# griosd/g3py

Hardware: AMD Instinct MI355X
Metric: GP logp+predict end-to-end (Gram+Cholesky+solves), N=32768 fp64: algorithmic TFLOP/s (higher is better)
Workload: dtype f64; 1 GPU; SE-kernel GaussianProcess, N=32768 d=4, M=1024 test points: Gram + blocked Cholesky + L^-1 y (logp) + cross-Gram + 1024-rhs trsm + posterior mean/variance; N=32768, d=4, M=1024, parallelism=1gpu

## Files before the change

### g3py_amd/csrc/g3_api.hip

```cpp
#include "g3_internal.h"
#include "g3_host.h"
#include <stdlib.h>

extern "C" int g3_version(void) { return 102; }

static int ctx_create_impl(int device, hipStream_t on_stream, g3_ctx** out);
extern "C" int g3_ctx_create(int device, g3_ctx** out) { return ctx_create_impl(device, nullptr, out); }
int g3i_ctx_create_on(int device, hipStream_t stream, g3_ctx** out) { return stream ? ctx_create_impl(device, stream, out) : -3; }
#include <time.h>
__global__ void probe_long_kernel(int iters) {
  for (int i = 0; i < iters; ++i) __builtin_amdgcn_s_sleep(127);
}
__global__ void probe_tiny_kernel(unsigned* out) {
  if (threadIdx.x == 0 && out) *out = 1u;
}
static double probe_now_us() {
  struct timespec ts;
  clock_gettime(CLOCK_MONOTONIC, &ts);
  return (double)ts.tv_sec * 1e6 + (double)ts.tv_nsec * 1e-3;
}
bool g3i_probe_pair(hipStream_t a, hipStream_t b, unsigned* scratch, double* tiny_us, double* long_us, int reps) {
  double best = 1e30, lbest = 1e30;
  for (int rep = 0; rep < reps; ++rep) {
    if (hipStreamSynchronize(a) != hipSuccess || hipStreamSynchronize(b) != hipSuccess) return false;
// ... 648 lines not shown
                          const void* delta, g3_dtype dt, void* K, int64_t ldk, void* invd, void* a, double out[6],
                          const g3_kernel_prog* prog_cross, const void* Xs, int64_t M, int64_t ldxs, void* mu,
                          void* ss) {
  const int64_t Np = g3_roundup(N, G3_LB), RB = 128, Mp = M > 0 ? g3_roundup(M, 128) : 0;
  const int64_t E = RB + Mp;
  const size_t es = g3_esize(dt);
  const double es_d = (double)es;
  char* rhs = (char*)K + (size_t)Np * ldk * es;
  char* Vp = rhs + (size_t)RB * ldk * es;
  int rc = G3_OK;
  const unsigned gflags = G3_GRAM_LOWER | G3_GRAM_SCRUB | G3_GRAM_PAD_EYE;
  auto build_rhs = [&]() -> int {
    const int r0 = pad_row_launch(ctx, rhs, ldk, delta, N, Np, RB, dt);
    if (r0) return r0;
    if (M > 0) {
      const int pr = g3i_prof_begin(ctx, G3_TAG_CROSS_GRAM, (double)(N + M) * d * es_d + (double)N * M * es_d);
      int r = g3_gram(ctx, prog_cross, Xs, M, ldxs, X, N, ldx, d, dt, Vp, ldk, Mp, Np, G3_GRAM_SCRUB);
      g3i_prof_end(ctx, pr);
      if (r) return r;
    }
    return G3_OK;
  };
  auto build = [&]() -> int {
    const int pr = g3i_prof_begin(ctx, G3_TAG_GRAM, (double)N * d * es_d + 0.5 * (double)N * (N + 1) * es_d);
    int r = g3_gram(ctx, prog, X, N, ldx, nullptr, 0, 0, d, dt, K, ldk, Np, Np, gflags);
    if (r) return r;
    r = g3_cov_lift(ctx, K, N, ldk, dt);
    g3i_prof_end(ctx, pr);
    if (r) return r;
    return build_rhs();
  };
  auto factor = [&]() -> int {
    const int pr = g3i_prof_begin(ctx, G3_TAG_POTRF, (double)N * N * N / 3.0 + (double)N * N * (1 + M));
    const int r = g3i_potrf_tall(ctx, K, Np, ldk, dt, invd, E);
    g3i_prof_end(ctx, pr);
    return r;
  };
  double st4[5];
  auto finish = [&]() -> int {
    const int pr = g3i_prof_begin(ctx, G3_TAG_REDUCE, 2.0 * N * M);
    g3_by_dtype(dt, [&](auto t) {
      using T = decltype(t);
      hipLaunchKernelGGL((logp_finish_kernel<T>), dim3(1), dim3(1024), 0, ctx->stream, (const T*)K, N, Np, ldk, (const T*)rhs, (T*)a,
                         ctx->d_stats, ctx->d_info);
    });
    G3_LAUNCH_CHECK();
    int r = G3_OK;
    if (M > 0 && (mu || ss)) r = rows_dot_ss_launch(ctx, Vp, M, N, ldk, a, dt, mu, ss);
    g3i_prof_end(ctx, pr);
    if (r) return r;
    r = fetch_stats(ctx, st4, 5);
    if (!r) { ctx->info_clean = true; ctx->info_sync = true; }
    return r;
  };
  rc = build();
  if (rc) return rc;
  rc = factor();
  if (rc) return rc;
  rc = finish();
  if (rc) return rc;
  int info = (int)st4[4];
  double tries = 0, fallback = 0;
  const int info0 = info;
  if (info != 0) {
    rc = build();
    if (rc) return rc;
// ... 118 lines not shown
  if (!a) return -15;
  if (!out) return -16;
  g3_kernel_prog first;
  if (g3i_validate_members(mp, batch, d, &first)) return -2;
  if (batch == 1)
    return gp_factor_impl(ctx, &first, X, N, ldx, d, delta, dt, K, ldk, invd, a, out, nullptr, nullptr, 0, 0, nullptr,
                          nullptr);
  const size_t sbytes = (size_t)batch * 4 * sizeof(double);
  g3_dev_members dm;
  int rc = g3i_upload_members(ctx, mp, batch, sbytes, g3i_coop_ctl_bytes(batch), &dm);
  if (rc) return rc;
  double* dstats = dm.stats;
  const int64_t wstride = Np * G3_LB;
  char* rhs = (char*)K + (size_t)Np * ldk * es;
  const bool small = Np <= 2 * G3_LB;
  int pr = g3i_prof_begin(ctx, G3_TAG_GRAM, (double)batch * ((double)N * d + 0.5 * (double)N * (N + 1)) * es);
  rc = g3i_gram_batched(ctx, dm.progs, &first, batch, X, N, ldx, d, dt, K, ldk, kstride, Np,
                        G3_GRAM_LOWER | G3_GRAM_SCRUB | G3_GRAM_PAD_EYE);
  if (!rc) rc = diag_stats_launch(ctx, K, N, ldk, dt, nullptr, 1, batch, kstride);
  if (!rc && !small) rc = pad_row_launch(ctx, rhs, ldk, delta, N, Np, RB, dt, batch, kstride, ldd);
  g3i_prof_end(ctx, pr);
  if (rc) return rc;
  pr = g3i_prof_begin(ctx, G3_TAG_POTRF, (double)batch * ((double)N * N * N / 3.0 + (double)N * N));
  if (small) {
    rc = g3i_small_factor_batched(ctx, K, ldk, kstride, invd, wstride, delta, ldd, a, Np, dstats, batch, N, Np, dt);
    g3i_prof_end(ctx, pr);
    if (!rc) rc = read_member_flags(ctx, batch, false);
  } else if (Np <= ctx->tune.coop_max_n && batch >= ctx->tune.coop_min_batch) {
    rc = g3i_coop_factor_batched(ctx, K, ldk, kstride, invd, wstride, (unsigned*)dm.tail, batch, Np, dt);
    g3i_prof_end(ctx, pr);
    if (!rc) rc = read_member_flags(ctx, batch, false);
  } else {
    g3_batch_scope mode(ctx, batch, kstride, wstride, invd, (size_t)batch * wstride * es);
    rc = g3i_potrf_tall(ctx, K, Np, ldk, dt, invd, RB);
    g3i_prof_end(ctx, pr);
    if (!rc) rc = read_member_flags(ctx, batch, true);
  }
  if (rc) return rc;
  if (!small) {
    G3_HIP(hipMemcpy2DAsync(a, (size_t)Np * es, rhs, (size_t)kstride * es, (size_t)Np * es, (size_t)batch,
                            hipMemcpyDeviceToDevice, ctx->stream));
    rc = g3i_logp_terms_dev(ctx, K, N, ldk, a, dt, dstats, batch, kstride, Np);
    if (rc) return rc;
  }
  double* hst = (double*)malloc(sbytes);
  if (!hst) return G3_ERR_NOMEM;
  if (hipMemcpyAsync(hst, dstats, sbytes, hipMemcpyDeviceToHost, ctx->stream) != hipSuccess ||
      hipStreamSynchronize(ctx->stream) != hipSuccess) {
    free(hst);
    snprintf(ctx->err, sizeof(ctx->err), "g3_gp_factor_batched: statistics copy failed");
    return G3_ERR_HIP;
  }
  int* infos = (int*)malloc(sizeof(int) * batch);
  if (!infos) { free(hst); return G3_ERR_NOMEM; }
  memcpy(infos, ctx->h_info, sizeof(int) * batch);
  for (int b = 0; b < batch && !rc; ++b) {
    double* o = out + 6 * b;
    if (infos[b] == 0) {
      o[0] = hst[4 * b]; o[1] = hst[4 * b + 1]; o[2] = hst[4 * b + 2];
      o[3] = 0; o[4] = 0; o[5] = 0;
    } else {
      g3_kernel_prog mine;
      mp.member(b, &mine);
      rc = gp_factor_impl(ctx, &mine, X, N, ldx, d, (const char*)delta + (size_t)b * ldd * es, dt,
                          (char*)K + (size_t)b * kstride * es, ldk, (char*)invd + (size_t)b * wstride * es,
                          (char*)a + (size_t)b * Np * es, o, nullptr, nullptr, 0, 0, nullptr, nullptr);
// ... 435 lines not shown
```

### g3py_amd/csrc/g3_gemm.hip

```cpp
#include "g3_internal.h"
#include <stdlib.h>

#include "g3_mfma.h"
#include "g3_host.h"

#include "g3_gemm_tile.h"


template <typename T, int BM, int BN, int WM, int WN, int NSTAGE>
__global__ void __launch_bounds__((BM / WM) * (BN / WN) * 64, ((BM / WM) * (BN / WN) >= 16 ? 1 : 2))
gemm_nt_kernel(T* C, int64_t ldc, const T* A, int64_t lda, const T* B, int64_t ldb,
               int K, T alpha, T beta, const int* __restrict__ info,
               int64_t bsC, int64_t bsA, int64_t bsB, const RasterTab tab) {
  C += (int64_t)blockIdx.y * bsC;
  A += (int64_t)blockIdx.y * bsA;
  B += (int64_t)blockIdx.y * bsB;
  if (info != nullptr) info += blockIdx.y;

  int bm, bn;
  {
    const int nwg = gridDim.x, id = blockIdx.x;
    const int q = nwg >> 3, r = nwg & 7, xcd = id & 7;
    const int v = (xcd < r ? xcd * (q + 1) : r * (q + 1) + (xcd - r) * q) + (id >> 3);
    int lo = 0, hi = tab.ngroups;
    while (hi - lo > 1) {
      const int mid = (lo + hi) >> 1;
      if (tab.g[mid].prefix <= v) lo = mid; else hi = mid;
    }
    const int w = v - tab.g[lo].prefix;
    const int rows = (int)tab.g[lo].nrows;
    bn = w / rows;
    bm = (int)tab.g[lo].row0 + (w - bn * rows);
  }
  const int doff = tab.diag_off;
  const bool lower_only = doff < G3_DENSE_OFF;
  const int m0 = bm * BM, n0 = bn * BN;
  if (lower_only && n0 > m0 + BM - 1 + doff) return;
  const int failed = (info != nullptr) ? *info : 0;
  int64_t brow = n0;
  if (tab.b_nb > 0) {
    const int sblk = n0 / tab.b_nb;
    brow = (int64_t)tab.b_blk[sblk] * tab.b_nb + (n0 - sblk * tab.b_nb);
  }
  extern __shared__ __attribute__((aligned(16))) char smem[];
  const int Kt = (tab.k_tri && n0 + BN < K) ? n0 + BN : K;
  gemm_tile<T, BM, BN, WM, WN, NSTAGE>(C, ldc, A + (int64_t)m0 * lda, lda, B + brow * ldb, ldb, Kt, alpha, beta, m0, n0,
                                       lower_only, doff, failed, smem);
}

template <typename T, int BM>
__global__ void __launch_bounds__(256, 2)
trsm_stripe_kernel(T* X, int64_t ldx, const T* L, int64_t ldl, const T* W, const int* __restrict__ info,
                   int64_t bsX, int64_t bsL, int64_t bsW, const TrsmOps ops) {
  X += (int64_t)blockIdx.y * bsX;
  L += (int64_t)blockIdx.y * bsL;
  W += (int64_t)blockIdx.y * bsW;
  if (info != nullptr) info += blockIdx.y;
  const int failed = (info != nullptr) ? *info : 0;
  if (failed != 0) return;
  extern __shared__ __attribute__((aligned(16))) char smem[];
  const int m0 = blockIdx.x * BM;
  for (int i = 0; i < ops.nops; ++i) {
    const auto o = ops.op[i];
    const T* gB = o.leaf ? W + (int64_t)o.brow * G3_LB * G3_LB : L + (int64_t)o.brow * ldl + o.bcol;
    gemm_tile<T, BM, 128, BM, 32, STAGES>(X, ldx, X + (int64_t)m0 * ldx + o.acol, ldx, gB, o.leaf ? (int64_t)G3_LB : ldl, o.k,
                                          o.leaf ? T(1) : T(-1), o.leaf ? T(0) : T(1), m0, o.col, false, G3_DENSE_OFF, 0, smem);
    __syncthreads();
  }
}


template <typename T, int BM, int BN, int WM, int WN, int NSTAGE>
static int launch_cfg(g3_ctx* ctx, void* C, int64_t ldc, const void* A, int64_t lda, const void* B,
                      int64_t ldb, int64_t k, double alpha, double beta, const GemmShape& sh) {
  constexpr int NT = (BM / WM) * (BN / WN) * 64;
  constexpr int LDS = NSTAGE * (BM + BN) * ROWB;
  auto kern = gemm_nt_kernel<T, BM, BN, WM, WN, NSTAGE>;
  static bool attr_set[G3_MAX_DEVICES] = {};
  const int dev_slot = ctx->device & (G3_MAX_DEVICES - 1);
  if (!attr_set[dev_slot]) {
    G3_HIP(hipFuncSetAttribute(reinterpret_cast<const void*>(kern),
                               hipFuncAttributeMaxDynamicSharedMemorySize, 160 * 1024));
    attr_set[dev_slot] = true;
  }
  RasterTab tab;
  const long long nv = build_raster<BM, BN>(sh, &tab);
  if (nv < 0) {
    snprintf(ctx->err, sizeof(ctx->err), "GEMM raster needs more than %d row groups", G3_RASTER_MAX);
    return G3_ERR_HIP;
  }
  if (nv == 0) return G3_OK;
  dim3 grid((unsigned)nv, (unsigned)g3_nbatch(ctx));
  int lds_req = LDS;
  if (ctx->tune.side_lds > LDS && (g3_on_bulk_stream(ctx) || ctx->bulk_role)) lds_req = ctx->tune.side_lds;
  const int tag = (BM == 128 && BN == 128) ? (nv >= 4096 ? G3_TAG_GEMM_BIG : G3_TAG_GEMM_MID) : G3_TAG_GEMM_SMALL;
  const double kmean = sh.k_tri ? 0.5 * ((double)k + (double)BN) : (double)k;
  const int pr = g3i_prof_begin(ctx, tag, 2.0 * shape_elems(sh) * kmean);
  if (FILE* lg = ctx->gemm_log)
    fprintf(lg, "gemm %d %d %d %lld %lld %lld %d %lld %.9e %d\n", BM, BN, NT / 64, (long long)sh.m, (long long)sh.n, (long long)k, sh.kind,
            nv, 2.0 * shape_elems(sh) * kmean, g3_on_bulk_stream(ctx) ? 1 : 0);
  hipLaunchKernelGGL(kern, grid, dim3(NT), lds_req, ctx->stream, (T*)C, ldc, (const T*)A, lda,
                     (const T*)B, ldb, (int)k, (T)alpha, (T)beta, ctx->d_info,
                     g3_bstride_of(ctx, C), g3_bstride_of(ctx, A), g3_bstride_of(ctx, B), tab);
  g3i_prof_end(ctx, pr);
  G3_LAUNCH_CHECK();
  return G3_OK;
}

template <typename T>
static int launch_t(g3_ctx* ctx, void* C, int64_t ldc, const void* A, int64_t lda, const void* B,
                    int64_t ldb, int64_t k, double alpha, double beta, const GemmShape& sh, int wide) {
  const int64_t blocks128 = (int64_t)(shape_elems(sh) / (128.0 * 128.0)) * g3_nbatch(ctx);
  bool all128 = sh.m % 128 == 0 && sh.n % 128 == 0;
  if (sh.kind == 2)
    for (int s = 0; s < sh.nseg; ++s) all128 = all128 && sh.seg_rows[s] % 128 == 0 && sh.seg_cols[s] % 128 == 0;
  if (wide) {
    if (sh.kind == 0 && sh.n % 128 == 0 && sh.m % 32 == 0)
      return launch_cfg<T, 32, 128, 32, 32, STAGES>(ctx, C, ldc, A, lda, B, ldb, k, alpha, beta, sh);
    snprintf(ctx->err, sizeof(ctx->err), "in-place panel GEMM needs n %% 128 == 0 and m %% 32 == 0 (m=%lld n=%lld)",
             (long long)sh.m, (long long)sh.n);
    return G3_ERR_HIP;
  }
  const int64_t big_min = ctx->tune.gemm_big_min;
  if (all128 && (blocks128 >= big_min || (blocks128 >= ctx->tune.gemm_big_min_k && k >= 1024 && big_min == 4096)))
    return launch_cfg<T, 128, 128, 64, 32, STAGES>(ctx, C, ldc, A, lda, B, ldb, k, alpha, beta, sh);
  return launch_cfg<T, 64, 64, 32, 32, STAGES>(ctx, C, ldc, A, lda, B, ldb, k, alpha, beta, sh);
}

static int launch_dt(g3_ctx* ctx, void* C, int64_t ldc, const void* A, int64_t lda, const void* B,
                     int64_t ldb, int64_t k, double alpha, double beta, g3_dtype dt, const GemmShape& sh, int wide) {
  return g3_by_dtype(dt, [&](auto t) { return launch_t<decltype(t)>(ctx, C, ldc, A, lda, B, ldb, k, alpha, beta, sh, wide); });
}

int g3i_gemm_nt_ex(g3_ctx* ctx, void* C, int64_t ldc, const void* A, int64_t lda, const void* B,
                   int64_t ldb, int64_t m, int64_t n, int64_t k, double alpha, double beta,
                   g3_dtype dt, int lower_only, int wide) {
  if (m == 0 || n == 0) return G3_OK;
  const GemmShape sh{lower_only ? 1 : 0, m, n, 0, 0, nullptr, nullptr, 0, nullptr, 0, nullptr, 0};
  return launch_dt(ctx, C, ldc, A, lda, B, ldb, k, alpha, beta, dt, sh, wide);
}

int g3i_gemm_nt(g3_ctx* ctx, void* C, int64_t ldc, const void* A, int64_t lda, const void* B,
                int64_t ldb, int64_t m, int64_t n, int64_t k, double alpha, double beta,
                g3_dtype dt, int lower_only) {
  return g3i_gemm_nt_ex(ctx, C, ldc, A, lda, B, ldb, m, n, k, alpha, beta, dt, lower_only, 0);
}

int g3i_gemm_nt_ktri(g3_ctx* ctx, void* C, int64_t ldc, const void* A, int64_t lda, const void* V, int64_t ldv, int64_t m, int64_t n,
                     double alpha, double beta, g3_dtype dt) {
  if (m == 0 || n == 0) return G3_OK;
  const GemmShape sh{0, m, n, 0, 0, nullptr, nullptr, 0, nullptr, 0, nullptr, 1};
  return launch_dt(ctx, C, ldc, A, lda, V, ldv, n, alpha, beta, dt, sh, 0);
}

int g3i_gemm_nt_trap(g3_ctx* ctx, void* C, int64_t ldc, const void* A, int64_t lda, const void* B,
                     int64_t ldb, int64_t m, int64_t n, int64_t k, double alpha, double beta,
                     g3_dtype dt, int64_t diag_off) {
  if (m == 0 || n == 0) return G3_OK;
  const GemmShape sh{1, m, n, diag_off, 0, nullptr, nullptr, 0, nullptr, 0, nullptr, 0};
  return launch_dt(ctx, C, ldc, A, lda, B, ldb, k, alpha, beta, dt, sh, 0);
}

template <typename T, int BM>
static int trsm_stripe_t(g3_ctx* ctx, const T* L, int64_t n, int64_t ldl, T* X, int64_t m, int64_t ldx, const T* W) {
  constexpr int LDS = STAGES * (BM + 128) * ROWB;
  auto kern = trsm_stripe_kernel<T, BM>;
  static bool attr_set[G3_MAX_DEVICES] = {};
  const int dev_slot = ctx->device & (G3_MAX_DEVICES - 1);
  if (!attr_set[dev_slot]) {
    G3_HIP(hipFuncSetAttribute(reinterpret_cast<const void*>(kern), hipFuncAttributeMaxDynamicSharedMemorySize, LDS));
    attr_set[dev_slot] = true;
  }
  TrsmOps ops;
  ops.nops = 0;
  trsm_ops_rec(&ops, 0, n);
  const int pr = g3i_prof_begin(ctx, G3_TAG_GEMM_SMALL, (double)m * (double)n * (double)n);
  if (FILE* lg = ctx->gemm_log)
    fprintf(lg, "trsm %d 128 4 %lld %lld %lld 0 %lld %.9e %d\n", BM, (long long)m, (long long)n, (long long)n, (long long)(m / BM),
            (double)m * (double)n * (double)n, g3_on_bulk_stream(ctx) ? 1 : 0);
  hipLaunchKernelGGL(kern, dim3((unsigned)(m / BM), (unsigned)g3_nbatch(ctx)), dim3(256), LDS, ctx->stream, X, ldx, L, ldl, W,
                     ctx->d_info, g3_bstride_of(ctx, X), g3_bstride_of(ctx, L), g3_bstride_of(ctx, W), ops);
  g3i_prof_end(ctx, pr);
  G3_LAUNCH_CHECK();
  return G3_OK;
}

int g3i_trsm_stripe(g3_ctx* ctx, const void* L, int64_t n, int64_t ldl, void* X, int64_t m, int64_t ldx, const void* W,
                    g3_dtype dt) {
  if (n > 1024 || n % G3_LB || m % 32 || m <= 0) return 1;
  const int64_t al = 16 / (int64_t)g3_esize(dt);
  if (ldx % al || ldl % al || (((uintptr_t)X | (uintptr_t)L | (uintptr_t)W) & 15)) return 1;
  const int64_t thin_max = ctx->tune.trsm_thin_max;
// ... 90 lines not shown
```

### g3py_amd/csrc/g3_host.h

```cpp
#pragma once
#include <stddef.h>
#include <stdint.h>
#include <stdlib.h>
#include <string.h>

#include <vector>

#include "g3hip.h"

#define G3H_LB 128

static inline int64_t g3h_roundup(int64_t n, int64_t m) { return (n + m - 1) / m * m; }

static inline int g3h_env_int(const char* name, int dflt) {
  const char* e = getenv(name);
  return e ? atoi(e) : dflt;
}

struct G3hTune {
  int64_t nb;
  int sb;
  int nb_tail;
  int nb_min;
  int nb_head;
  int side_lds;
  int64_t gemm_big_min;
  int64_t gemm_big_min_k;
  int64_t trsm_thin_max;
  int64_t trsm_wide_min;
  int64_t trsm_split_min;
  int64_t trsm_split_n;
  int stair_max;
  int gram_interpret;
  int grad_interpret;
  int gram_jit;
  int coop_max_n;
  int coop_min_batch;
  int coop_group;
  int probe;
};
#define G3H_STAIR_MAX 160
static inline G3hTune g3h_tune_from_env() {
  G3hTune t;
  const char* e = getenv("G3_NB");
  t.nb = e ? atoll(e) : 0;
  t.sb = g3h_env_int("G3_SB", 1);
  t.nb_tail = g3h_env_int("G3_NB_TAIL", 10);
  t.nb_min = g3h_env_int("G3_NB_MIN", 128);
  t.nb_head = g3h_env_int("G3_NB_HEAD", -1);
  t.side_lds = g3h_env_int("G3_SIDE_LDS", 54000);
  e = getenv("G3_GEMM_BIG_MIN");
  t.gemm_big_min = e ? atoll(e) : 4096;
  e = getenv("G3_GEMM_BIG_MIN_K");
  t.gemm_big_min_k = e ? atoll(e) : 1024;
  e = getenv("G3_TRSM_THIN_MAX");
  t.trsm_thin_max = e ? atoll(e) : 2048;
  e = getenv("G3_TRSM_WIDE_MIN");
  t.trsm_wide_min = e ? atoll(e) : 12288;
  e = getenv("G3_TRSM_SPLIT_MIN");
  t.trsm_split_min = e ? atoll(e) : 0;
  e = getenv("G3_TRSM_SPLIT_N");
  t.trsm_split_n = e ? atoll(e) : 512;
  const int sm = g3h_env_int("G3_STAIR_MAX", G3H_STAIR_MAX);
  t.stair_max = sm < 1 ? 1 : (sm > G3H_STAIR_MAX ? G3H_STAIR_MAX : sm);
  t.gram_interpret = g3h_env_int("G3_GRAM_NOFAST", 0) ? 1 : 0;
  t.grad_interpret = g3h_env_int("G3_GRAD_GENERIC", 0) ? 1 : 0;
  t.gram_jit = g3h_env_int("G3_GRAM_JIT", 1) ? 1 : 0;
  t.coop_max_n = g3h_env_int("G3_COOP_MAX_N", 1024);
  t.coop_min_batch = g3h_env_int("G3_COOP_MIN_BATCH", 200);
  t.coop_group = g3h_env_int("G3_COOP_GROUP", 0);
  t.probe = g3h_env_int("G3_PROBE", 1);
  return t;
}

static inline void g3h_panel_bounds(int64_t n, int64_t NB, int G, int batch, const G3hTune& tune, std::vector<int64_t>* bnd, std::vector<int>* grp) {
  const int taper = tune.nb_tail;
  const int wmin = tune.nb_min;
  const int64_t wlo = batch > 1 && wmin < 256 ? 256 : wmin;
  bnd->clear();
  grp->clear();
  if (NB < G3H_LB) NB = G3H_LB;
  if (G < 1) G = 1;
  const int head = tune.nb_head >= 0 ? tune.nb_head : (n <= 16384 ? 1 : 0);
  int64_t r0 = 0;
  int hstep = head;
  while (r0 < n) {
    int64_t w = NB;
    if (hstep > 0 && n >= 8 * NB) {
      w = NB >> hstep;
      if (w < G3H_LB) w = G3H_LB;
      --hstep;
    }
    if (taper) {
      const int64_t rem = n - r0;
      while (w > wlo && rem <= (int64_t)taper * w) w /= 2;
    }
    w = g3h_roundup(w, G3H_LB);
    bnd->push_back(r0);
    r0 += w;
  }
  bnd->push_back(n);
  const int nblk = (int)bnd->size() - 1;
  for (int k = 0; k < nblk; k += G) grp->push_back(k);
  grp->push_back(nblk);
}

constexpr int GROUP_M = 4;
constexpr int G3_RASTER_MAX = 160;
constexpr int G3_DENSE_OFF = 1 << 30;
struct RasterTab {
  int ngroups;
  int diag_off;
  struct Group {
    int prefix;
    unsigned short row0;
    unsigned short nrows;
  } g[G3_RASTER_MAX + 1];
  int b_nb;
  unsigned short b_blk[G3_RASTER_MAX];
  int k_tri;
};


struct GemmShape {
  int kind;
  int64_t m, n;
  int64_t off;
  int nseg;
  const int64_t* seg_rows;
  const int64_t* seg_cols;
  int64_t b_nb;
  const int32_t* b_perm;
  int nperm;
  const int64_t* seg_diag;
  int k_tri;
};

static inline double shape_elems(const GemmShape& sh) {
  if (sh.kind == 0) return (double)sh.m * (double)sh.n;
  if (sh.kind == 2) {
    double e = 0;
    for (int s = 0; s < sh.nseg; ++s) {
      e += (double)sh.seg_rows[s] * (double)sh.seg_cols[s];
      if (sh.seg_diag && sh.seg_diag[s] && sh.seg_cols[s] >= sh.seg_rows[s])
        e -= 0.5 * (double)sh.seg_rows[s] * ((double)sh.seg_rows[s] - 1.0);
    }
    return e;
  }
  int64_t i0 = sh.off < 0 ? -sh.off : 0;
  if (i0 > sh.m) i0 = sh.m;
  int64_t i1 = sh.n - 1 - sh.off;
  if (i1 < i0) i1 = i0;
  if (i1 > sh.m) i1 = sh.m;
  const double cnt = (double)(i1 - i0);
  const double tri = cnt * ((double)i0 + (double)sh.off + 1.0) + 0.5 * cnt * (cnt - 1.0);
  return tri + (double)(sh.m - i1) * (double)sh.n;
}

template <int BM, int BN>
static inline long long build_raster(const GemmShape& sh, RasterTab* tab) {
  const int64_t tiles_m = sh.m / BM;
  tab->diag_off = sh.kind == 1 ? (int)sh.off : G3_DENSE_OFF;
  int ng = 0;
  long long total = 0;
  auto push = [&](int64_t row_tile0, int64_t rows, int64_t nc) -> bool {
    if (rows <= 0 || nc <= 0) return true;
    if (ng >= G3_RASTER_MAX) return false;
    tab->g[ng].prefix = (int)total;
    tab->g[ng].row0 = (unsigned short)row_tile0;
    tab->g[ng].nrows = (unsigned short)rows;
    total += rows * nc;
    ++ng;
    return true;
  };
  if (sh.kind == 2) {
    int64_t rt = 0;
    int64_t ngroups_min = 0;
    for (int s = 0; s < sh.nseg; ++s) ngroups_min += (sh.seg_rows[s] / BM + GROUP_M - 1) / GROUP_M;
    const int64_t gh = ngroups_min <= G3_RASTER_MAX ? GROUP_M : GROUP_M * ((ngroups_min + G3_RASTER_MAX - 1) / G3_RASTER_MAX + 1);
    for (int s = 0; s < sh.nseg; ++s) {
      const int64_t st = sh.seg_rows[s] / BM, nc = sh.seg_cols[s] / BN;
      const bool dg = sh.seg_diag && sh.seg_diag[s] && sh.seg_cols[s] >= sh.seg_rows[s];
      const int64_t dcol0 = sh.seg_cols[s] - sh.seg_rows[s];
      for (int64_t t = 0; t < st; t += gh) {
        const int64_t rows = st - t < gh ? st - t : gh;
        int64_t ncg = nc;
        if (dg) {
          ncg = (dcol0 + (t + rows) * BM - 1) / BN + 1;
          if (ncg > nc) ncg = nc;
        }
        if (!push(rt + t, rows, ncg)) return -1;
      }
      rt += st;
    }
  } else {
    const int64_t tiles_n = sh.n / BN;
    int64_t gh = GROUP_M;
    if ((tiles_m + gh - 1) / gh > G3_RASTER_MAX) gh = (tiles_m + G3_RASTER_MAX - 1) / G3_RASTER_MAX;
    if (gh > 65535) return -1;
    for (int64_t t = 0; t < tiles_m; t += gh) {
      const int64_t rows = tiles_m - t < gh ? tiles_m - t : gh;
      int64_t nc = tiles_n;
      if (sh.kind == 1) {
        const int64_t lim = (t + rows) * BM - 1 + sh.off;
        nc = lim < 0 ? 0 : lim / BN + 1;
        if (nc > tiles_n) nc = tiles_n;
      }
      if (!push(t, rows, nc)) return -1;
    }
  }
  tab->ngroups = ng;
  tab->g[ng].prefix = (int)total;
  tab->g[ng].row0 = 0;
  tab->g[ng].nrows = 1;
  tab->k_tri = (sh.kind == 0 && sh.k_tri) ? 1 : 0;
  tab->b_nb = 0;
  if (sh.b_nb > 0 && sh.b_perm) {
    if (sh.nperm > G3_RASTER_MAX || sh.b_nb % BN) return -1;
    tab->b_nb = (int)sh.b_nb;
    for (int i = 0; i < sh.nperm; ++i) tab->b_blk[i] = (unsigned short)sh.b_perm[i];
  }
  return total;
}


constexpr int G3_TRSM_MAXOPS = 20;
struct TrsmOps {
  int nops;
  struct Op {
    int col;
    int acol;
    int k;
    int brow, bcol;
    int leaf;
  } op[G3_TRSM_MAXOPS];
};


static inline int64_t g3h_split_point(int64_t n) {
  int64_t g = G3H_LB;
  while (g * 2 <= n / 4 && g < 2048) g *= 2;
// ... 325 lines not shown
```

### g3py_amd/csrc/g3_internal.h

```cpp
#pragma once
#include <hip/hip_runtime.h>
#include <stdint.h>
#include <stdio.h>
#include <string.h>

#include "g3hip.h"
#include "g3_host.h"
#include "g3_reduce.h"

#define G3_LB 128

#define G3_PROG_SLOTS 8
struct g3_ctx {
  int device;
  hipStream_t stream;
  hipStream_t own_stream;
  hipStream_t side_stream;
  hipStream_t side_for;
  hipEvent_t* la_ev;
  int la_nev;
  bool in_sweep;
  G3hTune tune;
  unsigned long long gram_paths[3];
  unsigned long long grad_paths[3];
  FILE* gemm_log;
  bool info_clean;
  bool info_sync;
  hipStream_t info_stream;
  bool adopted;
  bool bulk_role;
  int batch;
  int64_t bstride, bstride_w;
  const char* bw_base;
  size_t bw_bytes;
  int64_t gram_diag_off;
  void* bbuf;
  size_t bbuf_bytes;
  int* d_info;
  double* d_stats;
  g3_kernel_prog* d_prog;
  hipEvent_t prog_ev[G3_PROG_SLOTS];
  bool prog_busy[G3_PROG_SLOTS];
  int prog_next, prog_last;
  hipStream_t prog_stream;
  int* h_info;
  double* h_stats;
  g3_kernel_prog* h_prog;
  void* invd;
  size_t invd_bytes;
  void* work;
  size_t work_bytes;
  bool prof_on;
  int prof_level;
  unsigned prof_skip;
  hipEvent_t* prof_ev;
  int prof_cap, prof_n;
  struct { int e0, e1, tag; double work; }* prof_rec;
  int prof_nrec;
  char err[512];
};

enum { G3_TAG_GEMM_BIG = 0, G3_TAG_GRAM = 1, G3_TAG_POTRF = 2, G3_TAG_TRSV = 3, G3_TAG_CROSS_GRAM = 4,
       G3_TAG_TRSM = 5, G3_TAG_REDUCE = 6, G3_TAG_GEMM_MID = 7, G3_TAG_GEMM_SMALL = 8, G3_TAG_LEAF = 9,
// ... 31 lines not shown
  ~g3_dev_guard() {
    if (switched && prev >= 0) (void)hipSetDevice(prev);
  }
  g3_dev_guard(const g3_dev_guard&) = delete;
  g3_dev_guard& operator=(const g3_dev_guard&) = delete;
};
#define G3_MAX_DEVICES 64

#define G3_MAX_BATCH 4096
static inline int g3_nbatch(const g3_ctx* ctx) { return ctx->batch > 1 ? ctx->batch : 1; }
static inline int64_t g3_bstride_of(const g3_ctx* ctx, const void* p) {
  if (ctx->batch <= 1) return 0;
  const char* c = (const char*)p;
  return (ctx->bw_base && c >= ctx->bw_base && c < ctx->bw_base + ctx->bw_bytes) ? ctx->bstride_w : ctx->bstride;
}

struct g3_batch_scope {
  g3_ctx* ctx;
  g3_batch_scope(g3_ctx* c, int batch, int64_t stride, int64_t stride_w, const void* w_base, size_t w_bytes) : ctx(c) {
    ctx->batch = batch;
    ctx->bstride = stride;
    ctx->bstride_w = stride_w;
    ctx->bw_base = (const char*)w_base;
    ctx->bw_bytes = w_bytes;
  }
  ~g3_batch_scope() {
    ctx->batch = 0;
    ctx->bw_base = nullptr;
  }
  g3_batch_scope(const g3_batch_scope&) = delete;
  g3_batch_scope& operator=(const g3_batch_scope&) = delete;
};

static inline bool g3_on_bulk_stream(const g3_ctx* ctx) { return ctx->stream == ctx->side_stream; }

int g3i_ensure_events(g3_ctx* ctx, int need);

struct g3_stream_scope {
  g3_ctx* ctx;
  hipStream_t prev;
  g3_stream_scope(g3_ctx* c, hipStream_t s) : ctx(c), prev(c->stream) { ctx->stream = s; }
  ~g3_stream_scope() { ctx->stream = prev; }
  g3_stream_scope(const g3_stream_scope&) = delete;
  g3_stream_scope& operator=(const g3_stream_scope&) = delete;
};

struct g3_sweep_scope {
  g3_ctx* ctx;
  hipStream_t chain, bulk;
  hipEvent_t ev;
  int rc;
  g3_sweep_scope(g3_ctx* c, hipStream_t bulk_, hipEvent_t ev_) : ctx(c), chain(c->stream), bulk(bulk_), ev(ev_) {
    if (bulk != chain) ctx->in_sweep = true;
    rc = wait(bulk, chain);
  }
  ~g3_sweep_scope() {
    if (bulk != chain) ctx->in_sweep = false;
  }
  int join() { return wait(chain, bulk); }
  g3_sweep_scope(const g3_sweep_scope&) = delete;
  g3_sweep_scope& operator=(const g3_sweep_scope&) = delete;

 private:
  int wait(hipStream_t waiter, hipStream_t on) {
    if (bulk == chain) return G3_OK;
    G3_HIP(hipEventRecord(ev, on));
    G3_HIP(hipStreamWaitEvent(waiter, ev, 0));
    return G3_OK;
  }
};

static inline size_t g3_esize(g3_dtype dt) { return dt == G3_F64 ? 8 : 4; }
static inline int64_t g3_roundup(int64_t n, int64_t m) { return (n + m - 1) / m * m; }

template <typename F>
static inline auto g3_by_dtype(g3_dtype dt, F&& f) {
  if (dt == G3_F64) return f(double());
  return f(float());
}

int g3i_ctx_create_on(int device, hipStream_t stream, g3_ctx** out);
int g3i_ensure_side_stream(g3_ctx* ctx);
void g3i_ctx_forget_stream(g3_ctx* ctx, hipStream_t s);
bool g3i_probe_pair(hipStream_t a, hipStream_t b, unsigned* scratch, double* tiny_us, double* long_us, int reps);

int g3i_gemm_nt(g3_ctx* ctx, void* C, int64_t ldc, const void* A, int64_t lda, const void* B,
                int64_t ldb, int64_t m, int64_t n, int64_t k, double alpha, double beta,
                g3_dtype dt, int lower_only);
int g3i_gemm_nt_ex(g3_ctx* ctx, void* C, int64_t ldc, const void* A, int64_t lda, const void* B,
                   int64_t ldb, int64_t m, int64_t n, int64_t k, double alpha, double beta,
                   g3_dtype dt, int lower_only, int wide);
int g3i_gemm_nt_ktri(g3_ctx* ctx, void* C, int64_t ldc, const void* A, int64_t lda, const void* V, int64_t ldv, int64_t m, int64_t n,
                     double alpha, double beta, g3_dtype dt);
int g3i_gemm_nt_trap(g3_ctx* ctx, void* C, int64_t ldc, const void* A, int64_t lda, const void* B,
                     int64_t ldb, int64_t m, int64_t n, int64_t k, double alpha, double beta,
                     g3_dtype dt, int64_t diag_off);
int g3i_gemm_nt_stair(g3_ctx* ctx, void* C, int64_t ldc, const void* A, int64_t lda, const void* B,
                      int64_t ldb, int64_t k, const int64_t* seg_rows, const int64_t* seg_cols, int nseg,
                      double alpha, double beta, g3_dtype dt, int64_t b_nb, const int32_t* b_perm, int nperm,
                      const int64_t* seg_diag = nullptr);
int g3i_trsm_stripe(g3_ctx* ctx, const void* L, int64_t n, int64_t ldl, void* X, int64_t m, int64_t ldx, const void* W,
                    g3_dtype dt);
int g3i_potrf(g3_ctx* ctx, void* A, int64_t n, int64_t ld, g3_dtype dt, void* invd);
int g3i_potrf_tall(g3_ctx* ctx, void* A, int64_t n, int64_t ld, g3_dtype dt, void* invd, int64_t E);
int g3i_trsm_rlt(g3_ctx* ctx, const void* L, int64_t n, int64_t ldl, void* B, int64_t m,
                 int64_t ldb, g3_dtype dt, const void* invd);
int g3i_trtri_blocks(g3_ctx* ctx, const void* L, int64_t n, int64_t ldl, g3_dtype dt, void* invd);
int g3i_trtri_full(g3_ctx* ctx, const void* L, int64_t n, const void* W, void* V, void* Vt, void* U, g3_dtype dt);
int g3i_reset_info(g3_ctx* ctx);
int g3i_read_info(g3_ctx* ctx, int* info_host);
bool g3i_info_known_zero(const g3_ctx* ctx);
int g3i_diag_stats_dev(g3_ctx* ctx, const void* A, int64_t n, int64_t ld, g3_dtype dt, double* out_dev);
int g3i_logp_terms_dev(g3_ctx* ctx, const void* L, int64_t n, int64_t ld, const void* a, g3_dtype dt, double* out_dev, int batch = 1,
                       int64_t lstride = 0, int64_t astride = 0);
int g3i_small_factor_batched(g3_ctx* ctx, void* K, int64_t ld, int64_t kstride, void* W, int64_t wstride, const void* delta, int64_t ldd,
                             void* a, int64_t astride, double* dstats, int batch, int64_t n, int64_t np, g3_dtype dt);
size_t g3i_coop_ctl_bytes(int batch);
int g3i_coop_group(const g3_ctx* ctx, int batch, int64_t np);
int g3i_coop_factor_batched(g3_ctx* ctx, void* K, int64_t ld, int64_t kstride, void* W, int64_t wstride, unsigned* ctl, int batch,
                            int64_t np, g3_dtype dt);
int g3i_diag_add(g3_ctx* ctx, void* A, int64_t n, int64_t ld, g3_dtype dt, double value);
int g3i_scale(g3_ctx* ctx, void* A, int64_t rows, int64_t cols, int64_t ld, g3_dtype dt, double factor);
int g3i_gram_grad(g3_ctx* ctx, const g3_kernel_prog* prog, const g3_grad_map* map, const void* X, int64_t N, int64_t ldx,
                  int d, g3_dtype dt, const void* G, int64_t ldg, const void* alpha, double* out_host,
                  int64_t row0 = 0, int64_t nrows = -1);
#define G3_GRAD_JIT_MAXSLOTS 40
hipFunction_t g3i_grad_jit_function(g3_ctx* ctx, const g3_kernel_prog* prog_host, int d, g3_dtype dt, int* nslots);
int g3i_gram_grad_batched(g3_ctx* ctx, const g3_kernel_prog* progs, int batch, const g3_grad_map* map, const void* X, int64_t N,
                          int64_t ldx, int d, g3_dtype dt, const void* G, int64_t ldg, int64_t gstride, const void* alpha,
// ... 63 lines not shown
```

### g3py_amd/csrc/g3_potrf.hip

```cpp
#include "g3_internal.h"
#include <vector>
#include "g3_host.h"
#include "g3_mfma.h"
#include "g3_gemm_tile.h"
#include <stdlib.h>

#include "g3_diag.h"

template <typename T>
__global__ void __launch_bounds__(512, 4)
potrf256_kernel(T* A, int64_t ld, T* W, int* info, int64_t row_base, int64_t a_batch, int64_t w_batch) {
  info += blockIdx.y;
  if (*info != 0) return;
  A += (int64_t)blockIdx.y * a_batch;
  W += (int64_t)blockIdx.y * w_batch;
  __shared__ DiagLds<T> S;
  const int lane = threadIdx.x & 63;
  const int wv = __builtin_amdgcn_readfirstlane((int)(threadIdx.x >> 6));
  const int w = wv < 4 ? wv : 11 - wv;
  switch (w) {
    case 0: potrf256_wave<T, 0>(A, ld, W, info, row_base, S, lane); break;
    case 1: potrf256_wave<T, 1>(A, ld, W, info, row_base, S, lane); break;
    case 2: potrf256_wave<T, 2>(A, ld, W, info, row_base, S, lane); break;
    case 3: potrf256_wave<T, 3>(A, ld, W, info, row_base, S, lane); break;
// ... 226 lines not shown
  ctx->work_bytes = bytes;
  return G3_OK;
}


template <typename T>
static int potrf_lookahead(g3_ctx* ctx, T* A, int64_t n, int64_t ld, T* W, int64_t NB, int G, g3_dtype dt, int64_t E) {
  const int64_t R = n + E;
  std::vector<int64_t> bnd;
  std::vector<int> gb;
  g3h_panel_bounds(n, NB, G, ctx->batch, ctx->tune, &bnd, &gb);
  const int nblk = (int)bnd.size() - 1, ngrp = (int)gb.size() - 1;
  int rc = g3i_ensure_events(ctx, 4 * ngrp + 1);
  if (rc) return rc;
  hipEvent_t* evG = ctx->la_ev;
  hipEvent_t* evB1 = ctx->la_ev + ngrp;
  hipEvent_t* evB2a = ctx->la_ev + 2 * ngrp;
  rc = g3i_ensure_side_stream(ctx);
  if (rc) return rc;
  hipStream_t sA = ctx->stream, sB = ctx->side_stream;
  auto r = [&](int k) { return k < nblk ? bnd[k] : n; };
  auto c = [&](int s) { return s < ngrp ? bnd[gb[s]] : n; };
  g3_sweep_scope sweep(ctx, sB, ctx->la_ev[4 * ngrp]);
  if (sweep.rc) return sweep.rc;
  auto panel = [&](int k) -> int {
    T* Akk = A + r(k) * ld + r(k);
    const int64_t w = r(k + 1) - r(k);
    int e = potrf_rec<T>(ctx, Akk, w, ld, W + (r(k) / LB) * LB * LB, r(k), dt);
    if (e) return e;
    if (r(k + 1) < R) e = trsm_rec<T>(ctx, Akk, w, ld, A + r(k + 1) * ld + r(k), R - r(k + 1), ld,
                                      W + (r(k) / LB) * LB * LB, dt);
    return e;
  };
  auto update = [&](int64_t row0, int64_t col0, int64_t col1, int64_t k0, int64_t k1) -> int {
    if (col1 <= col0 || row0 >= R || k1 <= k0) return G3_OK;
    return g3i_gemm_nt_trap(ctx, A + row0 * ld + col0, ld, A + row0 * ld + k0, ld, A + col0 * ld + k0, ld, R - row0,
                            col1 - col0, k1 - k0, -1.0, 1.0, dt, row0 - col0);
  };
  for (int s = 0; s < ngrp; ++s) {
    const int g0 = gb[s], g1 = gb[s + 1];
    if (s >= 1) {
      if (s >= 2) G3_HIP(hipStreamWaitEvent(sA, evB2a[s - 2], 0));
      rc = update(r(g0), r(g0), r(g0 + 1), c(s - 1), c(s));
      if (rc) return rc;
    }
    for (int j = g0; j < g1; ++j) {
      rc = panel(j);
      if (rc) return rc;
      if (j + 1 < g1) {
        if (j == g0 && s >= 1) G3_HIP(hipStreamWaitEvent(sA, evB1[s - 1], 0));
        rc = update(r(j + 1), r(j + 1), r(j + 2), r(j), r(j + 1));
        if (!rc && j + 2 < g1) rc = update(r(j + 2), r(j + 2), c(s + 1), r(j), r(j + 1));
        if (rc) return rc;
      }
    }
    G3_HIP(hipEventRecord(evG[s], sA));
    if (c(s + 1) < n) {
      G3_HIP(hipStreamWaitEvent(sB, evG[s], 0));
      g3_stream_scope on_bulk(ctx, sB);
      const int h0 = gb[s + 1];
      rc = update(r(h0 + 1), r(h0 + 1), c(s + 2), c(s), c(s + 1));
      if (rc) return rc;
      G3_HIP(hipEventRecord(evB1[s], sB));
      if (c(s + 2) < n) {
        const int q0 = gb[s + 2];
        rc = update(c(s + 2), c(s + 2), r(q0 + 1), c(s), c(s + 1));
        if (rc) return rc;
        G3_HIP(hipEventRecord(evB2a[s], sB));
        rc = update(r(q0 + 1), r(q0 + 1), n, c(s), c(s + 1));
        if (rc) return rc;
// ... 422 lines not shown
```

Baseline: 62.70 TFLOP/s.

## Use thin 16-row GEMM tiles for the single-row RHS block in tall Cholesky updates

During the tall Cholesky factorization the appended right-hand-side rows (at row n) only hold one live row, yet trailing updates computed a full 128-row tile band for them. The raster builder now carves that band out into thin 16-row tiles placed at the end of each XCD's schedule, and these are computed with a dedicated 16xBN gemm_tile path. This drops the wasted FLOPs and loads on the padded RHS rows. The cost is added raster/scheduling complexity and a non-inlined thin tile path, and it relies on only the first 16 of the 128 padded rows needing results.

Result: no change. 63.20 TFLOP/s (median of 6 runs) (+0.8%).

```diff
diff --git a/g3py_amd/csrc/g3_api.hip b/g3py_amd/csrc/g3_api.hip
--- a/g3py_amd/csrc/g3_api.hip
+++ b/g3py_amd/csrc/g3_api.hip
@@ -704,6 +704,7 @@
   };
   auto factor = [&]() -> int {
     const int pr = g3i_prof_begin(ctx, G3_TAG_POTRF, (double)N * N * N / 3.0 + (double)N * N * (1 + M));
+    g3_rhs_one_row_scope one_row(ctx);
     const int r = g3i_potrf_tall(ctx, K, Np, ldk, dt, invd, E);
     g3i_prof_end(ctx, pr);
     return r;
@@ -888,6 +889,7 @@
     if (!rc) rc = read_member_flags(ctx, batch, false);
   } else {
     g3_batch_scope mode(ctx, batch, kstride, wstride, invd, (size_t)batch * wstride * es);
+    g3_rhs_one_row_scope one_row(ctx);
     rc = g3i_potrf_tall(ctx, K, Np, ldk, dt, invd, RB);
     g3i_prof_end(ctx, pr);
     if (!rc) rc = read_member_flags(ctx, batch, true);
diff --git a/g3py_amd/csrc/g3_gemm.hip b/g3py_amd/csrc/g3_gemm.hip
--- a/g3py_amd/csrc/g3_gemm.hip
+++ b/g3py_amd/csrc/g3_gemm.hip
@@ -6,6 +6,13 @@
 
 #include "g3_gemm_tile.h"
 
+
+template <typename T, int BN, int NSTAGE>
+__device__ __noinline__ void gemm_tile_thin(T* C, int64_t ldc, const T* gA, int64_t lda, const T* gB, int64_t ldb, int K, T alpha,
+                                            T beta, int m0, int n0, bool lower_only, int doff, int failed) {
+  extern __shared__ __attribute__((aligned(16))) char smem[];
+  gemm_tile<T, 16, BN, 16, 16, NSTAGE>(C, ldc, gA, lda, gB, ldb, K, alpha, beta, m0, n0, lower_only, doff, failed, smem);
+}
 
 template <typename T, int BM, int BN, int WM, int WN, int NSTAGE>
 __global__ void __launch_bounds__((BM / WM) * (BN / WN) * 64, ((BM / WM) * (BN / WN) >= 16 ? 1 : 2))
@@ -19,9 +26,7 @@
 
   int bm, bn;
   {
-    const int nwg = gridDim.x, id = blockIdx.x;
-    const int q = nwg >> 3, r = nwg & 7, xcd = id & 7;
-    const int v = (xcd < r ? xcd * (q + 1) : r * (q + 1) + (xcd - r) * q) + (id >> 3);
+    const int v = g3h_virtual_tile((int)blockIdx.x, (int)gridDim.x, tab.thin_tiles);
     int lo = 0, hi = tab.ngroups;
     while (hi - lo > 1) {
       const int mid = (lo + hi) >> 1;
@@ -44,6 +49,14 @@
   }
   extern __shared__ __attribute__((aligned(16))) char smem[];
   const int Kt = (tab.k_tri && n0 + BN < K) ? n0 + BN : K;
+  constexpr bool THIN = (BM / WM) * (BN / WN) == BN / 16 && 128 % BM == 0;
+  if constexpr (THIN) {
+    if (m0 == tab.thin_row0) {
+      gemm_tile_thin<T, BN, NSTAGE>(C, ldc, A + (int64_t)m0 * lda, lda, B + brow * ldb, ldb, Kt, alpha, beta, m0, n0, lower_only,
+                                    doff, failed);
+      return;
+    }
+  }
   gemm_tile<T, BM, BN, WM, WN, NSTAGE>(C, ldc, A + (int64_t)m0 * lda, lda, B + brow * ldb, ldb, Kt, alpha, beta, m0, n0,
                                        lower_only, doff, failed, smem);
 }
@@ -110,7 +123,9 @@
 template <typename T>
 static int launch_t(g3_ctx* ctx, void* C, int64_t ldc, const void* A, int64_t lda, const void* B,
                     int64_t ldb, int64_t k, double alpha, double beta, const GemmShape& sh, int wide) {
-  const int64_t blocks128 = (int64_t)(shape_elems(sh) / (128.0 * 128.0)) * g3_nbatch(ctx);
+  GemmShape whole = sh;
+  whole.thin_row0 = -1;
+  const int64_t blocks128 = (int64_t)(shape_elems(whole) / (128.0 * 128.0)) * g3_nbatch(ctx);
   bool all128 = sh.m % 128 == 0 && sh.n % 128 == 0;
   if (sh.kind == 2)
     for (int s = 0; s < sh.nseg; ++s) all128 = all128 && sh.seg_rows[s] % 128 == 0 && sh.seg_cols[s] % 128 == 0;
@@ -155,9 +170,9 @@
 
 int g3i_gemm_nt_trap(g3_ctx* ctx, void* C, int64_t ldc, const void* A, int64_t lda, const void* B,
                      int64_t ldb, int64_t m, int64_t n, int64_t k, double alpha, double beta,
-                     g3_dtype dt, int64_t diag_off) {
-  if (m == 0 || n == 0) return G3_OK;
-  const GemmShape sh{1, m, n, diag_off, 0, nullptr, nullptr, 0, nullptr, 0, nullptr, 0};
+                     g3_dtype dt, int64_t diag_off, int64_t thin_row0) {
+  if (m == 0 || n == 0) return G3_OK;
+  const GemmShape sh{1, m, n, diag_off, 0, nullptr, nullptr, 0, nullptr, 0, nullptr, 0, thin_row0};
   return launch_dt(ctx, C, ldc, A, lda, B, ldb, k, alpha, beta, dt, sh, 0);
 }
 
diff --git a/g3py_amd/csrc/g3_host.h b/g3py_amd/csrc/g3_host.h
--- a/g3py_amd/csrc/g3_host.h
+++ b/g3py_amd/csrc/g3_host.h
@@ -38,6 +38,7 @@
   int coop_min_batch;
   int coop_group;
   int probe;
+  int rhs_thin;
 };
 #define G3H_STAIR_MAX 160
 static inline G3hTune g3h_tune_from_env() {
@@ -70,6 +71,7 @@
   t.coop_min_batch = g3h_env_int("G3_COOP_MIN_BATCH", 200);
   t.coop_group = g3h_env_int("G3_COOP_GROUP", 0);
   t.probe = g3h_env_int("G3_PROBE", 1);
+  t.rhs_thin = g3h_env_int("G3_RHS_THIN", 1) ? 1 : 0;
   return t;
 }
 
@@ -119,7 +121,29 @@
   int b_nb;
   unsigned short b_blk[G3_RASTER_MAX];
   int k_tri;
-};
+  int thin_row0;
+  int thin_tiles;
+};
+constexpr int G3_THIN_ROWS = 16;
+
+#if defined(__HIPCC__)
+#define G3H_RASTER_HD __host__ __device__
+#else
+#define G3H_RASTER_HD
+#endif
+G3H_RASTER_HD static inline int g3h_xcd_first(int n, int x) {
+  const int q = n >> 3, r = n & 7;
+  return x < r ? x * (q + 1) : r * (q + 1) + (x - r) * q;
+}
+G3H_RASTER_HD static inline int g3h_virtual_tile(int id, int nwg, int thin) {
+  const int xcd = id & 7, slot = id >> 3;
+  const int slots0 = g3h_xcd_first(nwg, xcd);
+  if (thin <= 0) return slots0 + slot;
+  const int thin0 = g3h_xcd_first(thin, xcd), nthin = g3h_xcd_first(thin, xcd + 1) - thin0;
+  const int nslots = g3h_xcd_first(nwg, xcd + 1) - slots0;
+  const int nfull = nslots - nthin;
+  return slot < nfull ? (slots0 - thin0) + slot : (nwg - thin) + thin0 + (slot - nfull);
+}
 
 
 struct GemmShape {
@@ -134,7 +158,24 @@
   int nperm;
   const int64_t* seg_diag;
   int k_tri;
-};
+  int64_t thin_row0 = -1;
+};
+
+static inline double g3h_trap_elems(int64_t rows, int64_t n, int64_t off) {
+  int64_t i0 = off < 0 ? -off : 0;
+  if (i0 > rows) i0 = rows;
+  int64_t i1 = n - 1 - off;
+  if (i1 < i0) i1 = i0;
+  if (i1 > rows) i1 = rows;
+  const double cnt = (double)(i1 - i0);
+  const double tri = cnt * ((double)i0 + (double)off + 1.0) + 0.5 * cnt * (cnt - 1.0);
+  return tri + (double)(rows - i1) * (double)n;
+}
+
+static inline int64_t g3h_thin_row0(const GemmShape& sh) {
+  if (sh.kind != 1 || sh.thin_row0 < 0 || sh.thin_row0 % 128 || sh.thin_row0 + 128 > sh.m) return -1;
+  return sh.thin_row0;
+}
 
 static inline double shape_elems(const GemmShape& sh) {
   if (sh.kind == 0) return (double)sh.m * (double)sh.n;
@@ -147,20 +188,19 @@
     }
     return e;
   }
-  int64_t i0 = sh.off < 0 ? -sh.off : 0;
-  if (i0 > sh.m) i0 = sh.m;
-  int64_t i1 = sh.n - 1 - sh.off;
-  if (i1 < i0) i1 = i0;
-  if (i1 > sh.m) i1 = sh.m;
-  const double cnt = (double)(i1 - i0);
-  const double tri = cnt * ((double)i0 + (double)sh.off + 1.0) + 0.5 * cnt * (cnt - 1.0);
-  return tri + (double)(sh.m - i1) * (double)sh.n;
+  const double all = g3h_trap_elems(sh.m, sh.n, sh.off);
+  const int64_t thin = g3h_thin_row0(sh);
+  if (thin < 0) return all;
+  return all - (g3h_trap_elems(thin + 128, sh.n, sh.off) - g3h_trap_elems(thin + G3_THIN_ROWS, sh.n, sh.off));
 }
 
 template <int BM, int BN>
 static inline long long build_raster(const GemmShape& sh, RasterTab* tab) {
   const int64_t tiles_m = sh.m / BM;
   tab->diag_off = sh.kind == 1 ? (int)sh.off : G3_DENSE_OFF;
+  const int64_t thin = (BM == 64 || BM == 128) ? g3h_thin_row0(sh) : -1;
+  tab->thin_row0 = (int)thin;
+  tab->thin_tiles = 0;
   int ng = 0;
   long long total = 0;
   auto push = [&](int64_t row_tile0, int64_t rows, int64_t nc) -> bool {
@@ -195,18 +235,31 @@
     }
   } else {
     const int64_t tiles_n = sh.n / BN;
+    const int64_t thin_t = thin >= 0 ? thin / BM : -1;
+    const int64_t gmax = thin_t >= 0 ? G3_RASTER_MAX - 2 : G3_RASTER_MAX;
     int64_t gh = GROUP_M;
-    if ((tiles_m + gh - 1) / gh > G3_RASTER_MAX) gh = (tiles_m + G3_RASTER_MAX - 1) / G3_RASTER_MAX;
+    if ((tiles_m + gh - 1) / gh > gmax) gh = (tiles_m + gmax - 1) / gmax;
     if (gh > 65535) return -1;
-    for (int64_t t = 0; t < tiles_m; t += gh) {
-      const int64_t rows = tiles_m - t < gh ? tiles_m - t : gh;
+    auto ncols = [&](int64_t t, int64_t live) {
       int64_t nc = tiles_n;
       if (sh.kind == 1) {
-        const int64_t lim = (t + rows) * BM - 1 + sh.off;
+        const int64_t lim = t * BM + live - 1 + sh.off;
         nc = lim < 0 ? 0 : lim / BN + 1;
         if (nc > tiles_n) nc = tiles_n;
       }
-      if (!push(t, rows, nc)) return -1;
+      return nc;
+    };
+    for (int64_t t = 0; t < tiles_m;) {
+      if (t == thin_t) { t += 128 / BM; continue; }
+      int64_t rows = tiles_m - t < gh ? tiles_m - t : gh;
+      if (t < thin_t && t + rows > thin_t) rows = thin_t - t;
+      if (!push(t, rows, ncols(t, rows * BM))) return -1;
+      t += rows;
+    }
+    if (thin_t >= 0) {
+      const long long before = total;
+      if (!push(thin_t, 1, ncols(thin_t, G3_THIN_ROWS))) return -1;
+      tab->thin_tiles = (int)(total - before);
     }
   }
   tab->ngroups = ng;
diff --git a/g3py_amd/csrc/g3_internal.h b/g3py_amd/csrc/g3_internal.h
--- a/g3py_amd/csrc/g3_internal.h
+++ b/g3py_amd/csrc/g3_internal.h
@@ -29,6 +29,7 @@
   hipStream_t info_stream;
   bool adopted;
   bool bulk_role;
+  bool rhs_one_row;
   int batch;
   int64_t bstride, bstride_w;
   const char* bw_base;
@@ -126,6 +127,14 @@
   g3_batch_scope& operator=(const g3_batch_scope&) = delete;
 };
 
+struct g3_rhs_one_row_scope {
+  g3_ctx* ctx;
+  explicit g3_rhs_one_row_scope(g3_ctx* c) : ctx(c) { ctx->rhs_one_row = ctx->tune.rhs_thin != 0; }
+  ~g3_rhs_one_row_scope() { ctx->rhs_one_row = false; }
+  g3_rhs_one_row_scope(const g3_rhs_one_row_scope&) = delete;
+  g3_rhs_one_row_scope& operator=(const g3_rhs_one_row_scope&) = delete;
+};
+
 static inline bool g3_on_bulk_stream(const g3_ctx* ctx) { return ctx->stream == ctx->side_stream; }
 
 int g3i_ensure_events(g3_ctx* ctx, int need);
@@ -188,7 +197,7 @@
                      double alpha, double beta, g3_dtype dt);
 int g3i_gemm_nt_trap(g3_ctx* ctx, void* C, int64_t ldc, const void* A, int64_t lda, const void* B,
                      int64_t ldb, int64_t m, int64_t n, int64_t k, double alpha, double beta,
-                     g3_dtype dt, int64_t diag_off);
+                     g3_dtype dt, int64_t diag_off, int64_t thin_row0 = -1);
 int g3i_gemm_nt_stair(g3_ctx* ctx, void* C, int64_t ldc, const void* A, int64_t lda, const void* B,
                       int64_t ldb, int64_t k, const int64_t* seg_rows, const int64_t* seg_cols, int nseg,
                       double alpha, double beta, g3_dtype dt, int64_t b_nb, const int32_t* b_perm, int nperm,
diff --git a/g3py_amd/csrc/g3_potrf.hip b/g3py_amd/csrc/g3_potrf.hip
--- a/g3py_amd/csrc/g3_potrf.hip
+++ b/g3py_amd/csrc/g3_potrf.hip
@@ -282,10 +282,11 @@
                                       W + (r(k) / LB) * LB * LB, dt);
     return e;
   };
+  const bool thin_rhs = ctx->rhs_one_row && E >= LB;
   auto update = [&](int64_t row0, int64_t col0, int64_t col1, int64_t k0, int64_t k1) -> int {
     if (col1 <= col0 || row0 >= R || k1 <= k0) return G3_OK;
     return g3i_gemm_nt_trap(ctx, A + row0 * ld + col0, ld, A + row0 * ld + k0, ld, A + col0 * ld + k0, ld, R - row0,
-                            col1 - col0, k1 - k0, -1.0, 1.0, dt, row0 - col0);
+                            col1 - col0, k1 - k0, -1.0, 1.0, dt, row0 - col0, thin_rhs && row0 <= n ? n - row0 : -1);
   };
   for (int s = 0; s < ngrp; ++s) {
     const int g0 = gb[s], g1 = gb[s + 1];
```
